# Gadersd/stable-diffusion-xl-burn

Hardware: AMD Instinct MI355X
Metric: images/sec SDXL-base 1024x1024 30-step CFG7.5 (whole job); UNet step ms p50 (higher is better)
Workload: dtype f16; 1 GPU; SDXL-base 1024x1024, n_steps=30 (31 CFG UNet step pairs), CFG 7.5, batch 1 prompt/GPU + VAE decode to u8 (BASELINE configs[1]); precision=f16, vae_dtype=f32_split, weights=synthetic seeded (random-init SDXL-base architecture), mix_classes=0, parallelism=replica x1, 1 prompt per GPU, weights broadcast once over RCCL, hipgraph=True, split_cfg=False, fused_xattn=True, pipelined_decode=False, prompts_per_call=1, full=False, library=stable-diffusion-xl-burn_amd/lib/libsdxl_mi355.so, debug_set=

## Files before the change

### stable-diffusion-xl-burn_amd/csrc/capi_ops.hip

```cpp
#include "capi_internal.h"
#include <algorithm>
#include <cmath>

using namespace sdxl;

namespace {
__global__ void transpose_pad_kernel(const float* src, int lds_, int rows, int C, void* dst, int dt, int ldd) {
  const size_t i = (size_t)blockIdx.x * blockDim.x + threadIdx.x;
  if (i >= (size_t)rows * C) return;
  const int r = i / C, c = i - (size_t)r * C;
  const float v = src[(size_t)r * lds_ + c];
  if (dt == DT_F16) reinterpret_cast<_Float16*>(dst)[(size_t)c * ldd + r] = (_Float16)v;
  else reinterpret_cast<float*>(dst)[(size_t)c * ldd + r] = v;
}
__global__ void causal_mask_kernel(float* out, int n) {
  const int i = blockIdx.x * blockDim.x + threadIdx.x;
  if (i >= n * n) return;
  const int r = i / n, c = i - r * n;
  out[i] = c > r ? -INFINITY : 0.f;
}

struct Operand { std::string name; std::vector<int> shape; int kind; const float* data = nullptr; float eps = 0.f; int ld = 0; };
using Operands = std::vector<Operand>;
void add_linear(Operands& o, const std::string& n, int K, int N, const float* w, const float* b, int ld = 0) {
// ... 101 lines not shown
  float* bsrc = (float*)tmp.get((size_t)Cout * sizeof(float));
  float* xsrc = (float*)tmp.get(M * Cin * sizeof(float));
  void* xi = tmp.get(M * Cin * 2);
  void* yo = tmp.get(M * Cout * 2);
  launch_synth_fill(wsrc, (size_t)Cout * K, 0x1234, 3.4641f / std::sqrt((float)K), 0.f, s);
  launch_synth_fill(bsrc, Cout, 0x99, 0.1f, 0.f, s);
  launch_synth_fill(xsrc, M * Cin, 0x777, 3.4641f, 0.f, s);
  launch_copy_rows(xsrc, DT_F32, Cin, xi, DT_F16, Cin, (int)M, Cin, s);
  const bool ln_in = (geglu & 2) != 0, st_out = (geglu & 4) != 0, cold = (geglu & 8) != 0;
  geglu &= 1;
  Operands ops;
  if (ksize == 1) add_linear(ops, "w", K, Cout, wsrc, bsrc);
  else add_conv(ops, "w", Cout, Cin, ksize, wsrc, bsrc);
  Packed pk(ops, DT_F16, s);
  Lin l = ksize == 1 ? pk.wb.linear("w", geglu != 0) : pk.wb.conv("w");
  Exec ex; ex.s = s; ex.cdt = DT_F16; ex.sdt = DT_F16;
  give_splitk_ws(ex, tmp, B, H * W, Cout, s);
  std::vector<const void*> wcopies(1, l.w), wfcopies(1, l.wf);
  if (cold) {
    const size_t wbytes = (size_t)l.Npad * l.Kpad * 2;
    const int nc = (int)std::min<size_t>(96, (size_t)(320u << 20) / wbytes + 1);
    for (int i = 1; i < nc; ++i)
      for (auto* img : {&wcopies, &wfcopies}) {
        void* c = img->front() ? tmp.get(wbytes) : nullptr;
        if (c) SDXL_HIP(hipMemcpyAsync(c, img->front(), wbytes, hipMemcpyDeviceToDevice, s));
        img->push_back(c);
      }
  }
  Epi e; e.act = geglu ? 1 : 0;
  if (ln_in) {
    SDXL_REQUIRE(ksize == 1 && Cin % 64 == 0, "ln bench needs a linear with K % 64 == 0");
    float* stat = (float*)tmp.get(M * (size_t)(Cin / 64) * 2 * sizeof(float));
    float* cs = (float*)tmp.get((size_t)l.Npad * sizeof(float));
    launch_synth_fill(stat, M * (size_t)(Cin / 64) * 2, 0x31, 0.5f, 64.0f, s);
    launch_synth_fill(cs, l.Npad, 0x32, 0.1f, 0.f, s);
    l.cs = cs; e.ln_stat = stat;
  }
  if (st_out) {
    SDXL_REQUIRE(!geglu && Cout % 64 == 0, "stat bench needs a plain N % 64 == 0 output");
    e.stat_out = (float*)tmp.get(M * (size_t)(Cout / 64) * 2 * sizeof(float));
  }
  const ConvGeom g{B, H, W, H, W, ksize, 1, ksize / 2, 0};
  const Act out(yo, geglu ? Cout / 2 : Cout, DT_F16);
  *avg_ms = time_launches(s, 3, iters, [&](int i) {
    l.w = wcopies[(size_t)i % wcopies.size()];
    l.wf = wfcopies[(size_t)i % wfcopies.size()];
    run_conv(ex, l, Act(xi, Cin, DT_F16), Cin, g, out, e);
  });
  API_END
}
int sdxl_bench_attention(sdxl_ctx* ctx, void* stream, int B, int H, int Nq, int Nk, int iters, float* avg_ms) {
  API_BEGIN
  SDXL_REQUIRE(ctx && avg_ms && iters > 0, "bad argument");
  use(ctx);
  hipStream_t s = pick(ctx, stream);
  Tmp tmp;
  const int C = H * 64, npad = (int)round_up(Nk, 64);
  float* src = (float*)tmp.get((size_t)B * std::max(Nq, npad) * C * sizeof(float));
  void* q = tmp.get((size_t)B * Nq * C * 2);
  void* k = tmp.get((size_t)B * Nk * C * 2);
  void* vt = tmp.get((size_t)B * C * npad * 2);
  void* o = tmp.get((size_t)B * Nq * C * 2);
  launch_synth_fill(src, (size_t)B * Nq * C, 0x51, 3.4641f, 0.f, s);
  launch_copy_rows(src, DT_F32, C, q, DT_F16, C, B * Nq, C, s);
  launch_synth_fill(src, (size_t)B * Nk * C, 0x52, 3.4641f, 0.f, s);
  launch_copy_rows(src, DT_F32, C, k, DT_F16, C, B * Nk, C, s);
  launch_synth_fill(src, (size_t)B * C * npad, 0x53, 3.4641f, 0.f, s);
  launch_copy_rows(src, DT_F32, npad, vt, DT_F16, npad, B * C, npad, s);
  AttnParams p = attn_params(q, k, vt, npad, o, C, DT_F16, B, H, Nq, Nk);
  give_xsplit_ws(p, tmp, s);
  *avg_ms = time_launches(s, 3, iters, [&](int) { launch_attention_d64(p, s); });
  API_END
}

int sdxl_qkv_attention(sdxl_ctx* ctx, void* stream, const float* q, const float* k, const float* v, const float* mask, int B,
                       int Nq, int Nk, int n_state, int n_head, int dtype, float* out) {
  API_BEGIN
  SDXL_REQUIRE(ctx && q && k && v && out, "null argument");
  SDXL_REQUIRE(n_head > 0 && n_state % n_head == 0, "State size must be a multiple of head size");
  use(ctx);
  hipStream_t s = pick(ctx, stream);
  int cdt, sdt; no_mix(dtype); dtypes(dtype, cdt, sdt);
  const int d = n_state / n_head, npad = (int)round_up(Nk, 64);
  const size_t es = dt_size(cdt);
  const float scale = (float)(1.0 / std::sqrt((double)d));
  Tmp tmp;
  if (cdt == DT_HL) {
    SDXL_REQUIRE(d == 64 && !mask, "sdxl_qkv_attention: the split-operand mode covers unmasked head-dim-64 attention");
    void* kh = tmp.get((size_t)B * Nk * n_state * 4);
    void* vth = tmp.get((size_t)B * n_state * npad * 4);
    launch_f32_to_hl(k, n_state, kh, n_state, (size_t)B * Nk, n_state, s);
    launch_f32_to_hl(stage_vt(tmp, v, B, Nk, n_state, DT_F32, npad, s), npad, vth, npad, (size_t)B * n_state, npad, s);
    const AttnParams p = attn_params(q, kh, vth, npad, out, n_state, DT_HL, B, n_head, Nq, Nk);
    SDXL_REQUIRE(launch_attention_d64_hl(p, s), "split-operand attention kernel refused an aligned shape");
  } else if (d == 64 || (d == 512 && cdt == DT_F16 && !mask)) {
    void* qd = tmp.get((size_t)B * Nq * n_state * es);
    void* kd = tmp.get((size_t)B * Nk * n_state * es);
    void* od = tmp.get((size_t)B * Nq * n_state * es);
    launch_copy_rows(q, DT_F32, n_state, qd, cdt, n_state, B * Nq, n_state, s);
    launch_copy_rows(k, DT_F32, n_state, kd, cdt, n_state, B * Nk, n_state, s);
    AttnParams p = attn_params(qd, kd, stage_vt(tmp, v, B, Nk, n_state, cdt, npad, s), npad, od, n_state, cdt, B, n_head, Nq, Nk, scale);
    p.mask = mask; p.ldmask = Nk;
    if (d == 64 && cdt == DT_F16 && !mask) give_xsplit_ws(p, tmp, s);
    if (d == 64) launch_attention_d64(p, s);
    else SDXL_REQUIRE(launch_attention_hd512(p, s), "wide-head attention kernel refused an aligned f16 shape");
    launch_copy_rows(od, cdt, n_state, out, DT_F32, n_state, B * Nq, n_state, s);
  } else {
    const int kt = cdt == DT_F16 ? 64 : 32;
    const int dpad = (int)round_up(d, kt), kpad = (int)round_up(Nk, kt);
    const int rows_k = (int)round_up(Nk, 128), rows_v = (int)round_up(d, 128);
    void* qh = tmp.get((size_t)Nq * dpad * es);
    void* kh = tmp.get((size_t)rows_k * dpad * es);
    void* vt = tmp.get((size_t)rows_v * kpad * es);
    float* S = (float*)tmp.get((size_t)Nq * Nk * sizeof(float));
    void* P = tmp.get((size_t)Nq * kpad * es);
    launch_fill_zero(qh, (size_t)Nq * dpad * es, s);
    launch_fill_zero(kh, (size_t)rows_k * dpad * es, s);
    launch_fill_zero(vt, (size_t)rows_v * kpad * es, s);
    Exec ex; ex.s = s; ex.cdt = cdt; ex.sdt = sdt;
    for (int b = 0; b < B; ++b)
      for (int h = 0; h < n_head; ++h) {
        const float* qs = q + (size_t)b * Nq * n_state + h * d;
        const float* ks = k + (size_t)b * Nk * n_state + h * d;
        const float* vs = v + (size_t)b * Nk * n_state + h * d;
        launch_copy_rows(qs, DT_F32, n_state, qh, cdt, dpad, Nq, d, s);
        launch_copy_rows(ks, DT_F32, n_state, kh, cdt, dpad, Nk, d, s);
        transpose_pad(vs, n_state, Nk, d, vt, cdt, kpad, s);
        Lin lk; lk.w = kh; lk.N = Nk; lk.K = dpad; lk.Kpad = dpad; lk.Npad = rows_k; lk.cin = dpad;
        run_linear(ex, lk, Act(qh, dpad, cdt), Nq, Act(S, Nk, DT_F32));
        launch_softmax_rows(S, Nk, P, cdt, kpad, Nq, Nk, kpad, scale, mask, Nk, Nq, s);
        Lin lv; lv.w = vt; lv.N = d; lv.K = Nk; lv.Kpad = kpad; lv.Npad = rows_v; lv.cin = Nk;
        run_linear(ex, lv, Act(P, kpad, cdt), Nq, Act(out + (size_t)b * Nq * n_state + h * d, n_state, DT_F32));
      }
  }
  SDXL_HIP(hipStreamSynchronize(s));
  API_END
}
int sdxl_attn_decoder_mask(sdxl_ctx* ctx, void* stream, int n, float* out) {
  API_BEGIN
  SDXL_REQUIRE(ctx && out && n > 0, "bad argument");
  use(ctx);
  hipLaunchKernelGGL(causal_mask_kernel, dim3((n * n + 255) / 256), dim3(256), 0, pick(ctx, stream), out, n);
  API_END
}

int sdxl_group_norm(sdxl_ctx* ctx, void* stream, const float* x, const float* gamma, const float* beta, int B, int C, int HW,
                    int n_group, float eps, int silu, int dtype, float* out) {
  API_BEGIN
  SDXL_REQUIRE(ctx && x && gamma && beta && out, "null argument");
  SDXL_REQUIRE(n_group > 0 && C % n_group == 0, "The number of channels must be divisible by the number of groups");
  SDXL_REQUIRE(C % 8 == 0 && n_group <= 256, "unsupported GroupNorm shape");
  use(ctx);
  hipStream_t s = pick(ctx, stream);
  int cdt, sdt; no_mix(dtype); dtypes(dtype, cdt, sdt); no_split(cdt, "sdxl_group_norm");
  Tmp tmp;
  void* xi = tmp.get((size_t)B * HW * C * dt_size(sdt));
  void* yo = tmp.get((size_t)B * HW * C * dt_size(cdt));
  float* part = (float*)tmp.get(groupnorm_workspace_floats(B, n_group) * sizeof(float));
  launch_nchw_to_nhwc(x, C * HW, xi, sdt, B, C, HW, C, 1.0f, s);
  GroupNormParams p{};
  p.X = xi; p.x_dt = sdt; p.ldx = C; p.Y = yo; p.y_dt = cdt; p.ldy = C; p.gamma = gamma; p.beta = beta; p.partial = part;
  p.B = B; p.HW = HW; p.C = C; p.G = n_group; p.eps = eps; p.silu = silu;
  launch_groupnorm(p, s);
  launch_nhwc_to_nchw(yo, cdt, C, out, B, C, HW, 1.0f, s);
  SDXL_HIP(hipStreamSynchronize(s));
  API_END
}
int sdxl_layer_norm(sdxl_ctx* ctx, void* stream, const float* x, const float* gamma, const float* beta, int rows, int C,
                    float eps, int dtype, float* out) {
  API_BEGIN
  SDXL_REQUIRE(ctx && x && gamma && beta && out, "null argument");
  SDXL_REQUIRE(C % 8 == 0, "unsupported LayerNorm width");
  use(ctx);
  hipStream_t s = pick(ctx, stream);
  int cdt, sdt; no_mix(dtype); dtypes(dtype, cdt, sdt); no_split(cdt, "sdxl_layer_norm");
  Tmp tmp;
  void* xi = tmp.get((size_t)rows * C * dt_size(sdt));
  void* yo = tmp.get((size_t)rows * C * dt_size(cdt));
  launch_copy_rows(x, DT_F32, C, xi, sdt, C, rows, C, s);
  LayerNormParams p{};
  p.X = xi; p.x_dt = sdt; p.ldx = C; p.Y = yo; p.y_dt = cdt; p.ldy = C; p.gamma = gamma; p.beta = beta; p.rows = rows; p.C = C; p.eps = eps;
  launch_layernorm(p, s);
  launch_copy_rows(yo, cdt, C, out, DT_F32, C, rows, C, s);
  SDXL_HIP(hipStreamSynchronize(s));
  API_END
}
int sdxl_conv2d(sdxl_ctx* ctx, void* stream, const float* x, const float* weight, const float* bias, int B, int Cin, int H,
                int W, int Cout, int ksize, int stride, int pad, int upsample, int dtype, float* out) {
  API_BEGIN
  SDXL_REQUIRE(ctx && x && weight && out, "null argument");
  use(ctx);
  hipStream_t s = pick(ctx, stream);
  int cdt, sdt;
  if (dtype == SDXL_DTYPE_F32_SPLIT) { cdt = DT_HL; sdt = DT_HL; }
  else { no_mix(dtype); dtypes(dtype, cdt, sdt); }
  SDXL_REQUIRE(cdt != DT_HL || Cin % 32 == 0, "SDXL_DTYPE_F32_SPLIT convolutions need Cin % 32 == 0");
  const int Hs = upsample ? 2 * H : H, Ws = upsample ? 2 * W : W;
  const int Ho = (Hs + 2 * pad - ksize) / stride + 1, Wo = (Ws + 2 * pad - ksize) / stride + 1;
  Operands ops;
  add_conv(ops, "conv", Cout, Cin, ksize, weight, bias);
  Packed pk(ops, cdt, s);
  const Lin l = pk.wb.conv("conv");
  Tmp tmp;
  void* xi = tmp.get((size_t)B * H * W * Cin * dt_size(sdt));
  float* yo = (float*)tmp.get((size_t)B * Ho * Wo * Cout * sizeof(float));
  Act xa(xi, Cin, sdt);
  if (cdt == DT_HL) {
    float* x32 = (float*)tmp.get((size_t)B * H * W * Cin * sizeof(float));
    float* sc = (float*)tmp.get(hl_scale_floats(B) * sizeof(float));
    launch_nchw_to_nhwc(x, Cin * H * W, x32, DT_F32, B, Cin, H * W, Cin, 1.0f, s);
    launch_f32_to_hl_scaled(x32, Cin, xi, Cin, (size_t)B * H * W, Cin, sc, s, B);
    xa.a_scale = hl_scale_inv(sc, B); xa.a_scale_n = B;
  } else launch_nchw_to_nhwc(x, Cin * H * W, xi, sdt, B, Cin, H * W, Cin, 1.0f, s);
  Exec ex; ex.s = s; ex.cdt = cdt; ex.sdt = sdt;
  give_splitk_ws(ex, tmp, B, Ho * Wo, Cout, s);
  run_conv(ex, l, xa, Cin, ConvGeom{B, H, W, Ho, Wo, ksize, stride, pad, upsample ? 1 : 0}, Act(yo, Cout, DT_F32));
  launch_nhwc_to_nchw(yo, DT_F32, Cout, out, B, Cout, Ho * Wo, 1.0f, s);
  SDXL_HIP(hipStreamSynchronize(s));
  API_END
}
int sdxl_conv2d_upsample_folded(sdxl_ctx* ctx, void* stream, const float* x, const float* weight, const float* bias, int B, int Cin, int H, int W,
                                int Cout, int dtype, int* folded, float* out) {
  API_BEGIN
  SDXL_REQUIRE(ctx && x && weight && out, "null argument");
  SDXL_REQUIRE(dtype == SDXL_DTYPE_F16 || dtype == SDXL_DTYPE_F32_SPLIT, "the folded upsample convolution exists in the f16 and the split-operand engines");
  use(ctx);
  hipStream_t s = pick(ctx, stream);
  const int cdt = dtype == SDXL_DTYPE_F16 ? DT_F16 : DT_HL, sdt = cdt;
  SDXL_REQUIRE(Cin % (cdt == DT_HL ? 32 : 64) == 0, "the folded upsample convolution needs whole k-tiles per tap (Cin % 64, split-operand: Cin % 32)");
  Operands ops;
  add_conv(ops, "conv", Cout, Cin, 3, weight, bias);
  Packed pk(ops, cdt, s);
  const Lin l = pk.wb.conv("conv", true);
  Tmp tmp;
  const size_t rows = (size_t)B * H * W;
  void* xi = tmp.get(rows * Cin * dt_size(sdt));
  float* yo = (float*)tmp.get(4 * rows * Cout * sizeof(float));
  Act xa(xi, Cin, sdt);
  if (cdt == DT_HL) {
    float* x32 = (float*)tmp.get(rows * Cin * sizeof(float));
    float* sc = (float*)tmp.get(hl_scale_floats(B) * sizeof(float));
    launch_nchw_to_nhwc(x, Cin * H * W, x32, DT_F32, B, Cin, H * W, Cin, 1.0f, s);
    launch_f32_to_hl_scaled(x32, Cin, xi, Cin, rows, Cin, sc, s, B);
    xa.a_scale = hl_scale_inv(sc, B); xa.a_scale_n = B;
  } else launch_nchw_to_nhwc(x, Cin * H * W, xi, sdt, B, Cin, H * W, Cin, 1.0f, s);
  Exec ex; ex.s = s; ex.cdt = cdt; ex.sdt = sdt;
  give_splitk_ws(ex, tmp, B, 4 * H * W, Cout, s);
  Epi e; e.fold = true;
  bool took = false; e.fold_done = &took;
  run_conv(ex, l, xa, Cin, ConvGeom{B, H, W, 2 * H, 2 * W, 3, 1, 1, 1}, Act(yo, Cout, DT_F32), e);
  if (folded) *folded = took ? 1 : 0;
  launch_nhwc_to_nchw(yo, DT_F32, Cout, out, B, Cout, 4 * H * W, 1.0f, s);
  SDXL_HIP(hipStreamSynchronize(s));
  API_END
}
int sdxl_linear(sdxl_ctx* ctx, void* stream, const float* x, const float* weight, const float* bias, int M, int K, int N,
                int geglu, int dtype, float* out) {
  API_BEGIN
  SDXL_REQUIRE(ctx && x && weight && out, "null argument");
  SDXL_REQUIRE(!geglu || (N % 32 == 0), "GEGLU width must be a multiple of 32");
  use(ctx);
  hipStream_t s = pick(ctx, stream);
  int cdt, sdt;
  if (dtype == SDXL_DTYPE_F32_SPLIT) { cdt = DT_HL; sdt = DT_HL; }
  else { no_mix(dtype); dtypes(dtype, cdt, sdt); }
  SDXL_REQUIRE(cdt != DT_HL || K % 32 == 0, "SDXL_DTYPE_F32_SPLIT linear layers need K % 32 == 0");
  Operands ops;
  add_linear(ops, "lin", K, N, weight, bias);
  Packed pk(ops, cdt, s);
  const Lin l = pk.wb.linear("lin", geglu != 0);
  Tmp tmp;
  void* xi = tmp.get((size_t)M * K * dt_size(sdt));
  Act xa(xi, K, sdt);
  if (cdt == DT_HL) {
    float* sc = (float*)tmp.get(hl_scale_floats(1) * sizeof(float));
    launch_f32_to_hl_scaled(x, K, xi, K, (size_t)M, K, sc, s, 1);
    xa.a_scale = hl_scale_inv(sc, 1);
  } else launch_copy_rows(x, DT_F32, K, xi, sdt, K, M, K, s);
  Exec ex; ex.s = s; ex.cdt = cdt; ex.sdt = sdt;
  give_splitk_ws(ex, tmp, 1, M, N, s);
  Epi e; e.act = geglu ? 1 : 0;
  run_linear(ex, l, xa, M, Act(out, geglu ? N / 2 : N, DT_F32), e);
  SDXL_HIP(hipStreamSynchronize(s));
  API_END
}
int sdxl_gemv(sdxl_ctx* ctx, void* stream, const float* x, const float* weight, const float* bias, const float* yadd, int Bm, int K, int N,
              int silu_in, int silu_out, int dtype, float* out) {
  API_BEGIN
  SDXL_REQUIRE(ctx && x && weight && out, "null argument");
  SDXL_REQUIRE(Bm >= 1 && K >= 1 && N >= 1, "gemv: Bm, K, N must be >= 1");
  SDXL_REQUIRE(dtype == SDXL_DTYPE_F32 || dtype == SDXL_DTYPE_F16 || dtype == SDXL_DTYPE_F32_SPLIT,
               "sdxl_gemv takes SDXL_DTYPE_F32, SDXL_DTYPE_F16 or SDXL_DTYPE_F32_SPLIT");
  use(ctx);
  hipStream_t s = pick(ctx, stream);
  const int cdt = dtype == SDXL_DTYPE_F16 ? DT_F16 : dtype == SDXL_DTYPE_F32_SPLIT ? DT_HL : DT_F32;
  Operands ops;
  add_linear(ops, "lin", K, N, weight, bias);
  Packed pk(ops, cdt, s);
  const Lin l = pk.wb.linear("lin", false, gemv_weight_dt(cdt));
  GemvParams p{};
  p.X = x; p.ldx = K; p.W = l.w; p.w_dt = l.dt >= 0 ? l.dt : cdt; p.Kpad = l.Kpad; p.bias = bias ? l.b : nullptr;
  p.Y = out; p.ldy = N; p.Yadd = yadd; p.Bm = Bm; p.N = l.N; p.K = l.K;
  p.silu_in = silu_in != 0; p.silu_out = silu_out != 0;
  (void)hipGetLastError();
  launch_gemv(p, s);
  SDXL_HIP(hipGetLastError());
  SDXL_HIP(hipStreamSynchronize(s));
// ... 254 lines not shown
```

### stable-diffusion-xl-burn_amd/csrc/norm.hip

```cpp
#include "kernels.h"
#include <stdexcept>
#include <type_traits>

namespace sdxl {

typedef _Float16 half_t;
typedef _Float16 half8 __attribute__((ext_vector_type(8)));
typedef float f32x4 __attribute__((ext_vector_type(4)));

template <typename XT> __device__ __forceinline__ void load8(const XT* p, float (&v)[8]);
template <> __device__ __forceinline__ void load8<half_t>(const half_t* p, float (&v)[8]) {
  half8 h = *reinterpret_cast<const half8*>(p);
#pragma unroll
  for (int j = 0; j < 8; ++j) v[j] = (float)h[j];
}
template <> __device__ __forceinline__ void load8<float>(const float* p, float (&v)[8]) {
  f32x4 a = *reinterpret_cast<const f32x4*>(p), b = *reinterpret_cast<const f32x4*>(p + 4);
#pragma unroll
  for (int j = 0; j < 4; ++j) { v[j] = a[j]; v[4 + j] = b[j]; }
}
template <typename YT> __device__ __forceinline__ void store8(YT* p, const float (&v)[8]);
template <> __device__ __forceinline__ void store8<half_t>(half_t* p, const float (&v)[8]) {
  half8 h;
#pragma unroll
  for (int j = 0; j < 8; ++j) h[j] = (half_t)v[j];
  asm volatile("global_store_dwordx4 %0, %1, off sc0 sc1\n\ts_nop 1" ::"v"(p), "v"(h) : "memory");
}
template <> __device__ __forceinline__ void store8<float>(float* p, const float (&v)[8]) {
  f32x4 a, b;
#pragma unroll
  for (int j = 0; j < 4; ++j) { a[j] = v[j]; b[j] = v[4 + j]; }
  *reinterpret_cast<f32x4*>(p) = a; *reinterpret_cast<f32x4*>(p + 4) = b;
}

struct hlout_t { float logical; };
template <typename YT> __device__ __forceinline__ void store8r(YT* row, int col, const float (&v)[8]) { store8<YT>(row + col, v); }
template <> __device__ __forceinline__ void store8r<hlout_t>(hlout_t* row, int col, const float (&v)[8]) {
  half8 hi, lo;
#pragma unroll
  for (int j = 0; j < 8; ++j) {
    float x = v[j];
    asm("" : "+v"(x));
    hi[j] = (half_t)x; lo[j] = (half_t)(x - (float)hi[j]);
  }
  half_t* b = reinterpret_cast<half_t*>(row) + ((col >> 4) << 5) + (col & 15);
  *reinterpret_cast<half8*>(b) = hi;
  *reinterpret_cast<half8*>(b + 16) = lo;
}

__device__ __forceinline__ void chan_merge(float& na, float& ma, float& m2a, float nb, float mb, float m2b) {
  if (nb == 0.f) return;
  const float n = na + nb;
  const float d = mb - ma;
  const float f = nb / n;
  ma = ma + d * f;
  m2a = m2a + m2b + d * d * na * f;
  na = n;
}

template <typename XT>
__global__ __launch_bounds__(256) void gn_stats_kernel(const GroupNormParams p) {
  extern __shared__ __attribute__((aligned(16))) float sm[];
  const int C = p.C, NV = C >> 3;
  const int VPR = NV < 256 ? NV : 256;
  const int RL = 256 / VPR;
  float* chMean = sm;
  float* chM2 = sm + C;
  float* tmpMean = sm + 2 * C;
  float* tmpM2 = tmpMean + RL * VPR * 8;
  float* tmpCnt = tmpM2 + RL * VPR * 8;
  const int tid = threadIdx.x;
  const int b = blockIdx.y, s = blockIdx.x;
  const int rps = (p.HW + p.nsplit - 1) / p.nsplit;
  const int row_begin = s * rps;
  const int row_end = min(p.HW, row_begin + rps);
  const int rl = tid / VPR, vl = tid - rl * VPR;
  const XT* X = reinterpret_cast<const XT*>(p.X) + (size_t)b * p.HW * p.ldx;
  const int npass = (NV + VPR - 1) / VPR;
  float total_rows = (float)max(0, row_end - row_begin);
  float amax = 0.f;
  const bool want_amax = p.absmax_out != nullptr;

  for (int pass = 0; pass < npass; ++pass) {
    const int vc = pass * VPR + vl;
    const bool active = rl < RL && vc < NV;
    float mean[8], m2[8], cnt = 0.f;
#pragma unroll
    for (int j = 0; j < 8; ++j) { mean[j] = 0.f; m2[j] = 0.f; }
    if (active) {
      float piv[8], s1[8], s2[8];
#pragma unroll
      for (int j = 0; j < 8; ++j) { piv[j] = 0.f; s1[j] = 0.f; s2[j] = 0.f; }
      int row = row_begin + rl;
      if (row < row_end) load8<XT>(X + (size_t)row * p.ldx + vc * 8, piv);
      for (; row + 3 * RL < row_end; row += 4 * RL) {
        float v[4][8];
#pragma unroll
        for (int u = 0; u < 4; ++u) load8<XT>(X + (size_t)(row + u * RL) * p.ldx + vc * 8, v[u]);
        cnt += 4.f;
#pragma unroll
        for (int u = 0; u < 4; ++u)
#pragma unroll
          for (int j = 0; j < 8; ++j) {
            const float d = v[u][j] - piv[j];
            s1[j] += d;
            s2[j] = fmaf(d, d, s2[j]);
          }
        if (want_amax) {
#pragma unroll
          for (int u = 0; u < 4; ++u)
#pragma unroll
            for (int j = 0; j < 8; ++j) amax = fmaxf(amax, fabsf(v[u][j]));
        }
      }
      for (; row < row_end; row += RL) {
        float v[8];
        load8<XT>(X + (size_t)row * p.ldx + vc * 8, v);
        cnt += 1.f;
#pragma unroll
        for (int j = 0; j < 8; ++j) {
          const float d = v[j] - piv[j];
          s1[j] += d;
          s2[j] = fmaf(d, d, s2[j]);
          if (want_amax) amax = fmaxf(amax, fabsf(v[j]));
        }
      }
      if (cnt > 0.f) {
        const float inv = 1.f / cnt;
#pragma unroll
        for (int j = 0; j < 8; ++j) {
          const float dm = s1[j] * inv;
          mean[j] = piv[j] + dm;
          m2[j] = fmaxf(s2[j] - s1[j] * dm, 0.f);
        }
      }
    }
    if (rl < RL) {
#pragma unroll
      for (int j = 0; j < 8; ++j) {
        tmpMean[(rl * VPR + vl) * 8 + j] = mean[j];
        tmpM2[(rl * VPR + vl) * 8 + j] = m2[j];
      }
      if (vl == 0) tmpCnt[rl] = cnt;
    }
    __syncthreads();
    if (rl == 0 && vc < NV) {
#pragma unroll
      for (int j = 0; j < 8; ++j) {
        float na = 0.f, ma = 0.f, qa = 0.f;
        for (int r = 0; r < RL; ++r)
          chan_merge(na, ma, qa, tmpCnt[r], tmpMean[(r * VPR + vl) * 8 + j], tmpM2[(r * VPR + vl) * 8 + j]);
        chMean[vc * 8 + j] = ma;
        chM2[vc * 8 + j] = qa;
      }
    }
    __syncthreads();
  }
  if (want_amax) {
#pragma unroll
    for (int o = 32; o > 0; o >>= 1) amax = fmaxf(amax, __shfl_xor(amax, o));
    __shared__ float wmax[4];
    if ((tid & 63) == 0) wmax[tid >> 6] = amax;
    __syncthreads();
    if (tid == 0) {
      float* slot = p.absmax_out + (size_t)b * kHlAbsBlocks;
      slot[s] = fmaxf(fmaxf(wmax[0], wmax[1]), fmaxf(wmax[2], wmax[3]));
      for (int k = s + p.nsplit; k < kHlAbsBlocks; k += p.nsplit) slot[k] = 0.f;
    }
  }
  const int cpg = C / p.G;
  if (tid < p.G) {
    float na = 0.f, ma = 0.f, qa = 0.f;
    if (total_rows > 0.f)
      for (int c = tid * cpg; c < (tid + 1) * cpg; ++c) chan_merge(na, ma, qa, total_rows, chMean[c], chM2[c]);
    float* out = p.partial + (((size_t)b * p.G + tid) * p.nsplit + s) * 3;
    out[0] = na; out[1] = ma; out[2] = qa;
  }
}

__global__ __launch_bounds__(256) void gn_finalize_kernel(const GroupNormParams p, float* stat) {
  const int lane = threadIdx.x & 63;
  const int i = blockIdx.x * 4 + (threadIdx.x >> 6);
  if (i >= p.B * p.G) return;
  const float* part = p.partial + (size_t)i * p.nsplit * 3;
  float na = 0.f, ma = 0.f, qa = 0.f;
  for (int s = lane; s < p.nsplit; s += 64) chan_merge(na, ma, qa, part[s * 3], part[s * 3 + 1], part[s * 3 + 2]);
#pragma unroll
  for (int o = 1; o < 64; o <<= 1) {
    const float nb = __shfl_xor(na, o), mb = __shfl_xor(ma, o), qb = __shfl_xor(qa, o);
    const float n = na + nb;
    if (n > 0.f) {
      const float d = mb - ma;
      const float f = nb / n;
      const float mnew = (lane & o) ? mb + (ma - mb) * (na / n) : ma + d * f;
      qa = qa + qb + d * d * na * f;
      ma = mnew;
    }
    na = n;
  }
  if (lane == 0) {
    stat[i * 2] = ma;
    stat[i * 2 + 1] = 1.0f / sqrtf(qa / na + (p.eps_ptr ? *p.eps_ptr : p.eps));
  }
}

template <typename XT, typename YT, int FIN>
__global__ __launch_bounds__(256) void gn_apply_kernel(const GroupNormParams p, const float* stat_in, int rows_per_block) {
  const int C = p.C, NV = C >> 3;
  const int VPR = NV < 256 ? NV : 256;
  const int RL = 256 / VPR;
  const int tid = threadIdx.x, b = blockIdx.y;
  __shared__ float sstat[512];
  if constexpr (FIN != 0) {
    const int tpg = 256 / p.G;
    const int g = tid / tpg, sub = tid - g * tpg;
    float na = 0.f, ma = 0.f, qa = 0.f;
    if constexpr (FIN == 1) {
      const float* part = p.partial + ((size_t)b * p.G + g) * p.nsplit * 3;
      for (int s = sub; s < p.nsplit; s += tpg) chan_merge(na, ma, qa, part[s * 3], part[s * 3 + 1], part[s * 3 + 2]);
    } else {
      typedef float f32x2 __attribute__((ext_vector_type(2)));
      const int cpg_ = C / p.G, total = p.chan_rt * cpg_;
      const f32x2* cp = reinterpret_cast<const f32x2*>(p.chan_part) + (size_t)b * p.chan_rt * C + g * cpg_;
      const float cnt = (float)p.chan_rows;
      for (int e0 = sub; e0 < total; e0 += 4 * tpg) {
        f32x2 v[4];
#pragma unroll
        for (int u = 0; u < 4; ++u) {
          const int e = e0 + u * tpg;
          const int rt = e / cpg_, cc = e - rt * cpg_;
          v[u] = e < total ? cp[(size_t)rt * C + cc] : f32x2{0.f, 0.f};
        }
#pragma unroll
        for (int u = 0; u < 4; ++u) chan_merge(na, ma, qa, e0 + u * tpg < total ? cnt : 0.f, v[u][0], v[u][1]);
      }
    }
    for (int o = 1; o < tpg; o <<= 1) {
      const float nb = __shfl_xor(na, o), mb = __shfl_xor(ma, o), qb = __shfl_xor(qa, o);
      const float n = na + nb;
      if (n > 0.f) {
        const float d = mb - ma;
        const float f = nb / n;
        const float mnew = (sub & o) ? mb + (ma - mb) * (na / n) : ma + d * f;
        qa = qa + qb + d * d * na * f;
        ma = mnew;
      }
      na = n;
    }
    if (sub == 0) {
      sstat[g * 2] = ma;
      sstat[g * 2 + 1] = 1.0f / sqrtf(qa / na + (p.eps_ptr ? *p.eps_ptr : p.eps));
    }
    __syncthreads();
  }
  const int rl = tid / VPR, vl = tid - rl * VPR;
  const int cpg = C / p.G;
  const int row0 = blockIdx.x * rows_per_block;
  const int row1 = min(p.HW, row0 + rows_per_block);
  const XT* X = reinterpret_cast<const XT*>(p.X) + (size_t)b * p.HW * p.ldx;
  YT* Y = reinterpret_cast<YT*>(p.Y) + (size_t)b * p.HW * p.ldy;
  const int npass = (NV + VPR - 1) / VPR;
  for (int pass = 0; pass < npass; ++pass) {
    const int vc = pass * VPR + vl;
    if (rl >= RL || vc >= NV) continue;
    float mean[8], scale[8], beta[8];
#pragma unroll
    for (int j = 0; j < 8; ++j) {
      const int c = vc * 8 + j;
      const int g = c / cpg;
      const float* st = FIN != 0 ? sstat + g * 2 : stat_in + ((size_t)b * p.G + g) * 2;
      mean[j] = st[0];
      scale[j] = st[1] * p.gamma[c];
      beta[j] = p.beta[c];
    }
    int row = row0 + rl;
    for (; row + RL < row1; row += 2 * RL) {
      float v[2][8];
#pragma unroll
      for (int u = 0; u < 2; ++u) load8<XT>(X + (size_t)(row + u * RL) * p.ldx + vc * 8, v[u]);
#pragma unroll
      for (int u = 0; u < 2; ++u) {
#pragma unroll
        for (int j = 0; j < 8; ++j) {
          float y = (v[u][j] - mean[j]) * scale[j] + beta[j];
          if (p.silu) y = y / (1.0f + __expf(-y));
          v[u][j] = y;
        }
        store8r<YT>(Y + (size_t)(row + u * RL) * p.ldy, vc * 8, v[u]);
      }
    }
    for (; row < row1; row += RL) {
      float v[8];
      load8<XT>(X + (size_t)row * p.ldx + vc * 8, v);
#pragma unroll
      for (int j = 0; j < 8; ++j) {
        float y = (v[j] - mean[j]) * scale[j] + beta[j];
        if (p.silu) y = y / (1.0f + __expf(-y));
        v[j] = y;
      }
      store8r<YT>(Y + (size_t)row * p.ldy, vc * 8, v);
    }
  }
}

static_assert(kGnMaxSplit <= kHlAbsBlocks, "one absmax slot per row split (GroupNormParams::absmax_out)");
int groupnorm_nsplit(int B, int HW, int C) {
  (void)B; (void)C;
  int n = HW / 32;
  if (n < 1) n = 1;
  if (n > kGnMaxSplit) n = kGnMaxSplit;
  return n;
}

void launch_groupnorm(const GroupNormParams& pin, hipStream_t s) {
  GroupNormParams p = pin;
  p.nsplit = groupnorm_nsplit(p.B, p.HW, p.C);
  const int NV = p.C >> 3;
  const int VPR = NV < 256 ? NV : 256;
  const int RL = 256 / VPR;
  const size_t lds_stats = (size_t)(2 * p.C + 2 * RL * VPR * 8 + RL) * sizeof(float);
  const bool fin = p.G <= 256 && (p.G & (p.G - 1)) == 0 && 256 / p.G <= 64;
  const bool from_producer = p.chan_part != nullptr;
  if (from_producer && !(fin && p.C % p.G == 0 && p.chan_rt >= 1 && p.chan_rows >= 1))
    throw std::runtime_error("groupnorm: producer statistics need a power-of-two group count");
  dim3 g1(p.nsplit, p.B);
  if (!from_producer) {
    if (p.x_dt == DT_F16) hipLaunchKernelGGL(gn_stats_kernel<half_t>, g1, dim3(256), lds_stats, s, p);
    else hipLaunchKernelGGL(gn_stats_kernel<float>, g1, dim3(256), lds_stats, s, p);
  }
  float* stat = p.partial + (size_t)p.B * p.G * kGnMaxSplit * 3;
  if (!fin) hipLaunchKernelGGL(gn_finalize_kernel, dim3((p.B * p.G + 3) / 4), dim3(256), 0, s, p, stat);
  int rows_per_block = (int)(((long)p.B * p.HW + 511) / 512);
  if (rows_per_block < 4 * RL) rows_per_block = 4 * RL;
  if (rows_per_block > p.HW) rows_per_block = p.HW;
  dim3 g2((p.HW + rows_per_block - 1) / rows_per_block, p.B);
#define GN_APPLY(XT, YT)                                                                                              \
  do {                                                                                                                \
    if (from_producer) hipLaunchKernelGGL((gn_apply_kernel<XT, YT, 2>), g2, dim3(256), 0, s, p, stat, rows_per_block); \
    else if (fin) hipLaunchKernelGGL((gn_apply_kernel<XT, YT, 1>), g2, dim3(256), 0, s, p, stat, rows_per_block);     \
    else hipLaunchKernelGGL((gn_apply_kernel<XT, YT, 0>), g2, dim3(256), 0, s, p, stat, rows_per_block);              \
  } while (0)
  if (p.x_dt == DT_F16 && p.y_dt == DT_F16) GN_APPLY(half_t, half_t);
  else if (p.x_dt == DT_F32 && p.y_dt == DT_F16) GN_APPLY(float, half_t);
  else if (p.x_dt == DT_F32 && p.y_dt == DT_F32) GN_APPLY(float, float);
  else if (p.x_dt == DT_F32 && p.y_dt == DT_HL) {
    if ((p.C & 15) != 0 || (p.ldy & 15) != 0) throw std::runtime_error("groupnorm: HL16 output needs C % 16 == 0 rows");
    GN_APPLY(float, hlout_t);
  } else if (p.x_dt == DT_F16 && p.y_dt == DT_F32) GN_APPLY(half_t, float);
  else throw std::runtime_error("groupnorm: unsupported dtype pair");
#undef GN_APPLY
}

template <typename XT, typename YT>
__global__ __launch_bounds__(256) void layernorm_kernel(const LayerNormParams p) {
  const int lane = threadIdx.x & 63;
  const int row = blockIdx.x * 4 + (threadIdx.x >> 6);
  if (row >= p.rows) return;
  const XT* x = reinterpret_cast<const XT*>(p.X) + (size_t)row * p.ldx;
  YT* y = reinterpret_cast<YT*>(p.Y) + (size_t)row * p.ldy;
  const int NV = p.C >> 3;
  float sum = 0.f;
  for (int vc = lane; vc < NV; vc += 64) {
    float v[8];
    load8<XT>(x + vc * 8, v);
#pragma unroll
    for (int j = 0; j < 8; ++j) sum += v[j];
  }
#pragma unroll
  for (int o = 32; o > 0; o >>= 1) sum += __shfl_xor(sum, o);
  const float mean = sum / (float)p.C;
  float sq = 0.f;
  for (int vc = lane; vc < NV; vc += 64) {
    float v[8];
    load8<XT>(x + vc * 8, v);
#pragma unroll
    for (int j = 0; j < 8; ++j) { const float u = v[j] - mean; sq += u * u; }
  }
#pragma unroll
  for (int o = 32; o > 0; o >>= 1) sq += __shfl_xor(sq, o);
  const float rstd = 1.0f / sqrtf(sq / (float)p.C + (p.eps_ptr ? *p.eps_ptr : p.eps));
  for (int vc = lane; vc < NV; vc += 64) {
    float v[8];
    load8<XT>(x + vc * 8, v);
    f32x4 g0 = *reinterpret_cast<const f32x4*>(p.gamma + vc * 8), g1 = *reinterpret_cast<const f32x4*>(p.gamma + vc * 8 + 4);
    f32x4 b0 = *reinterpret_cast<const f32x4*>(p.beta + vc * 8), b1 = *reinterpret_cast<const f32x4*>(p.beta + vc * 8 + 4);
#pragma unroll
    for (int j = 0; j < 4; ++j) {
      v[j] = (v[j] - mean) * rstd * g0[j] + b0[j];
      v[4 + j] = (v[4 + j] - mean) * rstd * g1[j] + b1[j];
    }
    store8r<YT>(y, vc * 8, v);
    if constexpr (std::is_same<YT, half_t>::value) {
      if (p.dup_scale != 0.f) {
#pragma unroll
        for (int j = 0; j < 8; ++j) { const float h = (float)(half_t)v[j]; v[j] = p.dup_scale > 0.f ? h * p.dup_scale : (v[j] - h) * -p.dup_scale; }
        store8r<YT>(y, p.C + vc * 8, v);
      }
    }
  }
}

template <typename XT, typename YT, int MAXV>
__global__ __launch_bounds__(256) void layernorm_cached_kernel(const LayerNormParams p) {
  const int lane = threadIdx.x & 63;
  const int row = blockIdx.x * 4 + (threadIdx.x >> 6);
  if (row >= p.rows) return;
  const XT* x = reinterpret_cast<const XT*>(p.X) + (size_t)row * p.ldx;
  YT* y = reinterpret_cast<YT*>(p.Y) + (size_t)row * p.ldy;
  const int NV = p.C >> 3;
  float v[MAXV][8];
  float sum = 0.f;
#pragma unroll
  for (int i = 0; i < MAXV; ++i) {
    const int vc = lane + 64 * i;
    if (vc < NV) {
      load8<XT>(x + vc * 8, v[i]);
#pragma unroll
      for (int j = 0; j < 8; ++j) sum += v[i][j];
    }
  }
#pragma unroll
  for (int o = 32; o > 0; o >>= 1) sum += __shfl_xor(sum, o);
  const float mean = sum / (float)p.C;
  float sq = 0.f;
#pragma unroll
  for (int i = 0; i < MAXV; ++i)
    if (lane + 64 * i < NV) {
#pragma unroll
      for (int j = 0; j < 8; ++j) { const float u = v[i][j] - mean; sq += u * u; }
    }
#pragma unroll
  for (int o = 32; o > 0; o >>= 1) sq += __shfl_xor(sq, o);
  const float rstd = 1.0f / sqrtf(sq / (float)p.C + (p.eps_ptr ? *p.eps_ptr : p.eps));
#pragma unroll
  for (int i = 0; i < MAXV; ++i) {
    const int vc = lane + 64 * i;
    if (vc < NV) {
      f32x4 g0 = *reinterpret_cast<const f32x4*>(p.gamma + vc * 8), g1 = *reinterpret_cast<const f32x4*>(p.gamma + vc * 8 + 4);
      f32x4 b0 = *reinterpret_cast<const f32x4*>(p.beta + vc * 8), b1 = *reinterpret_cast<const f32x4*>(p.beta + vc * 8 + 4);
      float o[8];
#pragma unroll
      for (int j = 0; j < 4; ++j) {
        o[j] = (v[i][j] - mean) * rstd * g0[j] + b0[j];
        o[4 + j] = (v[i][4 + j] - mean) * rstd * g1[j] + b1[j];
      }
      store8r<YT>(y, vc * 8, o);
      if constexpr (std::is_same<YT, half_t>::value) {
        if (p.dup_scale != 0.f) {
#pragma unroll
          for (int j = 0; j < 8; ++j) { const float h = (float)(half_t)o[j]; o[j] = p.dup_scale > 0.f ? h * p.dup_scale : (o[j] - h) * -p.dup_scale; }
          store8r<YT>(y, p.C + vc * 8, o);
        }
      }
    }
  }
}

void launch_layernorm(const LayerNormParams& p, hipStream_t s) {
  dim3 g((p.rows + 3) / 4);
  if (p.dup_scale != 0.f && (p.y_dt != DT_F16 || p.ldy < 2 * p.C)) throw std::runtime_error("layernorm: the duplicated output needs f16 rows of 2 C elements");
  if (p.y_dt == DT_HL) {
    if (p.x_dt != DT_F32 || (p.C & 15) != 0 || (p.ldy & 15) != 0) throw std::runtime_error("layernorm: HL16 output needs fp32 input and C % 16 == 0 rows");
    if (p.C <= 8 * 64 * 3) hipLaunchKernelGGL((layernorm_cached_kernel<float, hlout_t, 3>), g, dim3(256), 0, s, p);
    else hipLaunchKernelGGL((layernorm_kernel<float, hlout_t>), g, dim3(256), 0, s, p);
    return;
  }
  if (p.C <= 8 * 64 * 3) {
    if (p.x_dt == DT_F16 && p.y_dt == DT_F16) hipLaunchKernelGGL((layernorm_cached_kernel<half_t, half_t, 3>), g, dim3(256), 0, s, p);
    else if (p.x_dt == DT_F32 && p.y_dt == DT_F16) hipLaunchKernelGGL((layernorm_cached_kernel<float, half_t, 3>), g, dim3(256), 0, s, p);
    else if (p.x_dt == DT_F32 && p.y_dt == DT_F32) hipLaunchKernelGGL((layernorm_cached_kernel<float, float, 3>), g, dim3(256), 0, s, p);
    else hipLaunchKernelGGL((layernorm_cached_kernel<half_t, float, 3>), g, dim3(256), 0, s, p);
    return;
  }
  if (p.x_dt == DT_F16 && p.y_dt == DT_F16) hipLaunchKernelGGL((layernorm_kernel<half_t, half_t>), g, dim3(256), 0, s, p);
  else if (p.x_dt == DT_F32 && p.y_dt == DT_F16) hipLaunchKernelGGL((layernorm_kernel<float, half_t>), g, dim3(256), 0, s, p);
  else if (p.x_dt == DT_F32 && p.y_dt == DT_F32) hipLaunchKernelGGL((layernorm_kernel<float, float>), g, dim3(256), 0, s, p);
  else hipLaunchKernelGGL((layernorm_kernel<half_t, float>), g, dim3(256), 0, s, p);
}

}
```

Before: 1.452 images/sec.

## Restructure GroupNorm apply with LDS affine tables, early loads, and templated SiLU

The GroupNorm apply kernel now builds per-channel mean, scale and beta tables in LDS and walks rows with a flattened thread-to-(row,vec) mapping. It issues the first X loads and the partial-stat loads before the statistics merge, so memory latency overlaps the reduction. SiLU becomes a template parameter, with a fast exp2/rcp path for f16 outputs. The stats kernel gains an 8-row unrolled walk, and the C API stops rejecting the split-f32 dtype for group_norm. The cost is dynamic LDS sized by C, a hard channel-count limit, and more register pressure.

New measurement: 1.460 images/sec, median of 6. No clear change (+0.6%).

```diff
diff --git a/stable-diffusion-xl-burn_amd/csrc/capi_ops.hip b/stable-diffusion-xl-burn_amd/csrc/capi_ops.hip
--- a/stable-diffusion-xl-burn_amd/csrc/capi_ops.hip
+++ b/stable-diffusion-xl-burn_amd/csrc/capi_ops.hip
@@ -277,7 +277,8 @@
   SDXL_REQUIRE(C % 8 == 0 && n_group <= 256, "unsupported GroupNorm shape");
   use(ctx);
   hipStream_t s = pick(ctx, stream);
-  int cdt, sdt; no_mix(dtype); dtypes(dtype, cdt, sdt); no_split(cdt, "sdxl_group_norm");
+  int cdt, sdt; no_mix(dtype); dtypes(dtype, cdt, sdt);
+  SDXL_REQUIRE(cdt != DT_HL || C % 16 == 0, "sdxl_group_norm: SDXL_DTYPE_F32_SPLIT needs C % 16 == 0");
   Tmp tmp;
   void* xi = tmp.get((size_t)B * HW * C * dt_size(sdt));
   void* yo = tmp.get((size_t)B * HW * C * dt_size(cdt));
diff --git a/stable-diffusion-xl-burn_amd/csrc/norm.hip b/stable-diffusion-xl-burn_amd/csrc/norm.hip
--- a/stable-diffusion-xl-burn_amd/csrc/norm.hip
+++ b/stable-diffusion-xl-burn_amd/csrc/norm.hip
@@ -93,38 +93,32 @@
       for (int j = 0; j < 8; ++j) { piv[j] = 0.f; s1[j] = 0.f; s2[j] = 0.f; }
       int row = row_begin + rl;
       if (row < row_end) load8<XT>(X + (size_t)row * p.ldx + vc * 8, piv);
-      for (; row + 3 * RL < row_end; row += 4 * RL) {
-        float v[4][8];
-#pragma unroll
-        for (int u = 0; u < 4; ++u) load8<XT>(X + (size_t)(row + u * RL) * p.ldx + vc * 8, v[u]);
-        cnt += 4.f;
-#pragma unroll
-        for (int u = 0; u < 4; ++u)
-#pragma unroll
-          for (int j = 0; j < 8; ++j) {
-            const float d = v[u][j] - piv[j];
-            s1[j] += d;
-            s2[j] = fmaf(d, d, s2[j]);
+      auto walk = [&](auto nu) {
+        constexpr int NU = decltype(nu)::value;
+        for (; row + (NU - 1) * RL < row_end; row += NU * RL) {
+          float v[NU][8];
+#pragma unroll
+          for (int u = 0; u < NU; ++u) load8<XT>(X + (size_t)(row + u * RL) * p.ldx + vc * 8, v[u]);
+          cnt += (float)NU;
+#pragma unroll
+          for (int u = 0; u < NU; ++u)
+#pragma unroll
+            for (int j = 0; j < 8; ++j) {
+              const float d = v[u][j] - piv[j];
+              s1[j] += d;
+              s2[j] = fmaf(d, d, s2[j]);
+            }
+          if (want_amax) {
+#pragma unroll
+            for (int u = 0; u < NU; ++u)
+#pragma unroll
+              for (int j = 0; j < 8; ++j) amax = fmaxf(amax, fabsf(v[u][j]));
           }
-        if (want_amax) {
-#pragma unroll
-          for (int u = 0; u < 4; ++u)
-#pragma unroll
-            for (int j = 0; j < 8; ++j) amax = fmaxf(amax, fabsf(v[u][j]));
         }
-      }
-      for (; row < row_end; row += RL) {
-        float v[8];
-        load8<XT>(X + (size_t)row * p.ldx + vc * 8, v);
-        cnt += 1.f;
-#pragma unroll
-        for (int j = 0; j < 8; ++j) {
-          const float d = v[j] - piv[j];
-          s1[j] += d;
-          s2[j] = fmaf(d, d, s2[j]);
-          if (want_amax) amax = fmaxf(amax, fabsf(v[j]));
-        }
-      }
+      };
+      walk(std::integral_constant<int, 8>{});
+      walk(std::integral_constant<int, 4>{});
+      walk(std::integral_constant<int, 1>{});
       if (cnt > 0.f) {
         const float inv = 1.f / cnt;
 #pragma unroll
@@ -204,36 +198,101 @@
   }
 }
 
-template <typename XT, typename YT, int FIN>
+template <typename XT> struct Raw8;
+template <> struct Raw8<half_t> {
+  half8 h;
+  __device__ __forceinline__ void load(const half_t* p) { h = *reinterpret_cast<const half8*>(p); }
+  __device__ __forceinline__ void get(float (&v)[8]) const {
+#pragma unroll
+    for (int j = 0; j < 8; ++j) v[j] = (float)h[j];
+  }
+};
+template <> struct Raw8<float> {
+  f32x4 a, b;
+  __device__ __forceinline__ void load(const float* p) { a = *reinterpret_cast<const f32x4*>(p); b = *reinterpret_cast<const f32x4*>(p + 4); }
+  __device__ __forceinline__ void get(float (&v)[8]) const {
+#pragma unroll
+    for (int j = 0; j < 4; ++j) { v[j] = a[j]; v[4 + j] = b[j]; }
+  }
+};
+
+template <bool FAST> __device__ __forceinline__ float silu(float y) {
+  if constexpr (FAST) return y * __builtin_amdgcn_rcpf(1.0f + __builtin_amdgcn_exp2f(y * -1.44269504088896340736f));
+  else return y / (1.0f + __expf(-y));
+}
+
+template <typename XT, typename YT, int FIN, bool SILU>
 __global__ __launch_bounds__(256) void gn_apply_kernel(const GroupNormParams p, const float* stat_in, int rows_per_block) {
+  extern __shared__ __attribute__((aligned(16))) float sm[];
   const int C = p.C, NV = C >> 3;
-  const int VPR = NV < 256 ? NV : 256;
-  const int RL = 256 / VPR;
   const int tid = threadIdx.x, b = blockIdx.y;
-  __shared__ float sstat[512];
+  f32x4* tM = reinterpret_cast<f32x4*>(sm);
+  f32x4* tS = tM + 2 * NV;
+  f32x4* tB = tS + 2 * NV;
+  float* sstat = sm + 3 * C;
+  f32x4* spare = tM + 6 * NV + ((p.G + 1) >> 1);
+  const int row0 = blockIdx.x * rows_per_block;
+  const int nrows = min(p.HW, row0 + rows_per_block) - row0;
+  const XT* X = reinterpret_cast<const XT*>(p.X) + ((size_t)b * p.HW + row0) * p.ldx;
+  YT* Y = reinterpret_cast<YT*>(p.Y) + ((size_t)b * p.HW + row0) * p.ldy;
+  const int dr = 256 / NV, dv = 256 - dr * NV;
+  int row = tid / NV, vc = tid - row * NV;
+  Raw8<XT> raw[4];
+  int rr[4], cc[4];
+  auto load4 = [&]() {
+#pragma unroll
+    for (int u = 0; u < 4; ++u) {
+      rr[u] = row; cc[u] = vc;
+      raw[u].load(X + (size_t)min(row, nrows - 1) * p.ldx + vc * 8);
+      vc += dv; row += dr;
+      if (vc >= NV) { vc -= NV; ++row; }
+    }
+  };
+  constexpr int NB = 4;
+  typedef float f32x2 __attribute__((ext_vector_type(2)));
+  const int cpg = C / p.G;
+  const int tpg = FIN != 0 ? 256 / p.G : 256;
+  const int g = tid / tpg, sub = tid - g * tpg;
+  const int total = FIN == 1 ? p.nsplit : p.chan_rt * cpg;
+  float pn[NB], pm[NB], pq[NB];
+  auto load_entries = [&](int e0) {
+#pragma unroll
+    for (int u = 0; u < NB; ++u) {
+      const int e = min(e0 + u * tpg, total - 1);
+      if constexpr (FIN == 1) {
+        const float* part = p.partial + (((size_t)b * p.G + g) * p.nsplit + e) * 3;
+        pn[u] = part[0]; pm[u] = part[1]; pq[u] = part[2];
+      } else {
+        const int rt = e / cpg;
+        const f32x2 v = reinterpret_cast<const f32x2*>(p.chan_part)[((size_t)b * p.chan_rt + rt) * C + g * cpg + (e - rt * cpg)];
+        pn[u] = (float)p.chan_rows; pm[u] = v[0]; pq[u] = v[1];
+      }
+    }
+  };
+  constexpr int NQ = 3;
+  const int nq = C >> 2;
+  f32x4 ga[NQ], be[NQ];
+  auto load_affine = [&](int q0) {
+#pragma unroll
+    for (int u = 0; u < NQ; ++u) {
+      const int q = min(q0 + u * 256, nq - 1);
+      ga[u] = reinterpret_cast<const f32x4*>(p.gamma)[q];
+      be[u] = reinterpret_cast<const f32x4*>(p.beta)[q];
+    }
+  };
+  if constexpr (FIN != 0) load_entries(sub);
+  float eps = p.eps;
+  if constexpr (FIN != 0) { if (p.eps_ptr) eps = *p.eps_ptr; }
+  load4();
+  load_affine(tid);
   if constexpr (FIN != 0) {
-    const int tpg = 256 / p.G;
-    const int g = tid / tpg, sub = tid - g * tpg;
     float na = 0.f, ma = 0.f, qa = 0.f;
-    if constexpr (FIN == 1) {
-      const float* part = p.partial + ((size_t)b * p.G + g) * p.nsplit * 3;
-      for (int s = sub; s < p.nsplit; s += tpg) chan_merge(na, ma, qa, part[s * 3], part[s * 3 + 1], part[s * 3 + 2]);
-    } else {
-      typedef float f32x2 __attribute__((ext_vector_type(2)));
-      const int cpg_ = C / p.G, total = p.chan_rt * cpg_;
-      const f32x2* cp = reinterpret_cast<const f32x2*>(p.chan_part) + (size_t)b * p.chan_rt * C + g * cpg_;
-      const float cnt = (float)p.chan_rows;
-      for (int e0 = sub; e0 < total; e0 += 4 * tpg) {
-        f32x2 v[4];
-#pragma unroll
-        for (int u = 0; u < 4; ++u) {
-          const int e = e0 + u * tpg;
-          const int rt = e / cpg_, cc = e - rt * cpg_;
-          v[u] = e < total ? cp[(size_t)rt * C + cc] : f32x2{0.f, 0.f};
-        }
-#pragma unroll
-        for (int u = 0; u < 4; ++u) chan_merge(na, ma, qa, e0 + u * tpg < total ? cnt : 0.f, v[u][0], v[u][1]);
-      }
+    for (int e0 = sub;;) {
+#pragma unroll
+      for (int u = 0; u < NB; ++u) chan_merge(na, ma, qa, e0 + u * tpg < total ? pn[u] : 0.f, pm[u], pq[u]);
+      e0 += NB * tpg;
+      if (e0 >= total) break;
+      load_entries(e0);
     }
     for (int o = 1; o < tpg; o <<= 1) {
       const float nb = __shfl_xor(na, o), mb = __shfl_xor(ma, o), qb = __shfl_xor(qa, o);
@@ -249,57 +308,53 @@
     }
     if (sub == 0) {
       sstat[g * 2] = ma;
-      sstat[g * 2 + 1] = 1.0f / sqrtf(qa / na + (p.eps_ptr ? *p.eps_ptr : p.eps));
+      sstat[g * 2 + 1] = 1.0f / sqrtf(qa / na + eps);
     }
     __syncthreads();
   }
-  const int rl = tid / VPR, vl = tid - rl * VPR;
-  const int cpg = C / p.G;
-  const int row0 = blockIdx.x * rows_per_block;
-  const int row1 = min(p.HW, row0 + rows_per_block);
-  const XT* X = reinterpret_cast<const XT*>(p.X) + (size_t)b * p.HW * p.ldx;
-  YT* Y = reinterpret_cast<YT*>(p.Y) + (size_t)b * p.HW * p.ldy;
-  const int npass = (NV + VPR - 1) / VPR;
-  for (int pass = 0; pass < npass; ++pass) {
-    const int vc = pass * VPR + vl;
-    if (rl >= RL || vc >= NV) continue;
-    float mean[8], scale[8], beta[8];
-#pragma unroll
-    for (int j = 0; j < 8; ++j) {
-      const int c = vc * 8 + j;
-      const int g = c / cpg;
-      const float* st = FIN != 0 ? sstat + g * 2 : stat_in + ((size_t)b * p.G + g) * 2;
-      mean[j] = st[0];
-      scale[j] = st[1] * p.gamma[c];
-      beta[j] = p.beta[c];
-    }
-    int row = row0 + rl;
-    for (; row + RL < row1; row += 2 * RL) {
-      float v[2][8];
-#pragma unroll
-      for (int u = 0; u < 2; ++u) load8<XT>(X + (size_t)(row + u * RL) * p.ldx + vc * 8, v[u]);
-#pragma unroll
-      for (int u = 0; u < 2; ++u) {
-#pragma unroll
-        for (int j = 0; j < 8; ++j) {
-          float y = (v[u][j] - mean[j]) * scale[j] + beta[j];
-          if (p.silu) y = y / (1.0f + __expf(-y));
-          v[u][j] = y;
-        }
-        store8r<YT>(Y + (size_t)(row + u * RL) * p.ldy, vc * 8, v[u]);
-      }
-    }
-    for (; row < row1; row += RL) {
+  for (int q0 = tid;;) {
+#pragma unroll
+    for (int u = 0; u < NQ; ++u) {
+      const int q = q0 + u * 256, c = 4 * min(q, nq - 1);
+      const int g0 = c / cpg, r = c - g0 * cpg;
+      f32x4 mu, sc;
+#pragma unroll
+      for (int j = 0; j < 4; ++j) {
+        const int gc = g0 + (r + j >= cpg) + (r + j >= 2 * cpg) + (r + j >= 3 * cpg);
+        const float* st = FIN != 0 ? sstat + gc * 2 : stat_in + ((size_t)b * p.G + gc) * 2;
+        mu[j] = st[0];
+        sc[j] = st[1] * ga[u][j];
+      }
+      const int i = (q & 1) * NV + (q >> 1);
+      *(q < nq ? tM + i : spare) = mu;
+      *(q < nq ? tS + i : spare) = sc;
+      *(q < nq ? tB + i : spare) = be[u];
+    }
+    q0 += NQ * 256;
+    if (q0 >= nq) break;
+    load_affine(q0);
+  }
+  __syncthreads();
+  for (;;) {
+#pragma unroll
+    for (int u = 0; u < 4; ++u) {
+      if (rr[u] >= nrows) continue;
+      const f32x4 m0 = tM[cc[u]], m1 = tM[NV + cc[u]], s0 = tS[cc[u]], s1 = tS[NV + cc[u]], b0 = tB[cc[u]], b1 = tB[NV + cc[u]];
       float v[8];
-      load8<XT>(X + (size_t)row * p.ldx + vc * 8, v);
-#pragma unroll
-      for (int j = 0; j < 8; ++j) {
-        float y = (v[j] - mean[j]) * scale[j] + beta[j];
-        if (p.silu) y = y / (1.0f + __expf(-y));
-        v[j] = y;
-      }
-      store8r<YT>(Y + (size_t)row * p.ldy, vc * 8, v);
-    }
+      raw[u].get(v);
+#pragma unroll
+      for (int j = 0; j < 4; ++j) {
+        v[j] = (v[j] - m0[j]) * s0[j] + b0[j];
+        v[4 + j] = (v[4 + j] - m1[j]) * s1[j] + b1[j];
+      }
+      if constexpr (SILU) {
+#pragma unroll
+        for (int j = 0; j < 8; ++j) v[j] = silu<std::is_same<YT, half_t>::value>(v[j]);
+      }
+      store8r<YT>(Y + (size_t)rr[u] * p.ldy, cc[u] * 8, v);
+    }
+    if (row >= nrows) break;
+    load4();
   }
 }
 
@@ -331,14 +386,20 @@
   float* stat = p.partial + (size_t)p.B * p.G * kGnMaxSplit * 3;
   if (!fin) hipLaunchKernelGGL(gn_finalize_kernel, dim3((p.B * p.G + 3) / 4), dim3(256), 0, s, p, stat);
   int rows_per_block = (int)(((long)p.B * p.HW + 511) / 512);
-  if (rows_per_block < 4 * RL) rows_per_block = 4 * RL;
+  if (rows_per_block < (512 + NV - 1) / NV) rows_per_block = (512 + NV - 1) / NV;
   if (rows_per_block > p.HW) rows_per_block = p.HW;
   dim3 g2((p.HW + rows_per_block - 1) / rows_per_block, p.B);
-#define GN_APPLY(XT, YT)                                                                                              \
-  do {                                                                                                                \
-    if (from_producer) hipLaunchKernelGGL((gn_apply_kernel<XT, YT, 2>), g2, dim3(256), 0, s, p, stat, rows_per_block); \
-    else if (fin) hipLaunchKernelGGL((gn_apply_kernel<XT, YT, 1>), g2, dim3(256), 0, s, p, stat, rows_per_block);     \
-    else hipLaunchKernelGGL((gn_apply_kernel<XT, YT, 0>), g2, dim3(256), 0, s, p, stat, rows_per_block);              \
+  const size_t lds_apply = (size_t)(3 * p.C + ((2 * p.G + 3) & ~3) + 4) * sizeof(float);
+  if (lds_apply > 64 * 1024) throw std::runtime_error("groupnorm: the per-channel table of C > 5376 channels does not fit the apply kernel's LDS");
+#define GN_APPLY2(XT, YT, SILU)                                                                                                        \
+  do {                                                                                                                                 \
+    if (from_producer) hipLaunchKernelGGL((gn_apply_kernel<XT, YT, 2, SILU>), g2, dim3(256), lds_apply, s, p, stat, rows_per_block);  \
+    else if (fin) hipLaunchKernelGGL((gn_apply_kernel<XT, YT, 1, SILU>), g2, dim3(256), lds_apply, s, p, stat, rows_per_block);       \
+    else hipLaunchKernelGGL((gn_apply_kernel<XT, YT, 0, SILU>), g2, dim3(256), lds_apply, s, p, stat, rows_per_block);                \
+  } while (0)
+#define GN_APPLY(XT, YT)                                                  \
+  do {                                                                    \
+    if (p.silu) GN_APPLY2(XT, YT, true); else GN_APPLY2(XT, YT, false);   \
   } while (0)
   if (p.x_dt == DT_F16 && p.y_dt == DT_F16) GN_APPLY(half_t, half_t);
   else if (p.x_dt == DT_F32 && p.y_dt == DT_F16) GN_APPLY(float, half_t);
@@ -348,6 +409,7 @@
     GN_APPLY(float, hlout_t);
   } else if (p.x_dt == DT_F16 && p.y_dt == DT_F32) GN_APPLY(half_t, float);
   else throw std::runtime_error("groupnorm: unsupported dtype pair");
+#undef GN_APPLY2
 #undef GN_APPLY
 }
 
```
